# drprojects/DeepViewAgg

Measured on NVIDIA H100. Metric: Mpoints/s through view-agg fwd+bwd, higher is better.
Workload: dtype f32

## Files before the change

deepviewagg_b200/csrc/view_attention_lane.cu:

```cuda
#include "view_attention.cuh"

namespace dva {

constexpr int kLaneWarps = 4;
constexpr uint32_t kFull = 0xffffffffu;

struct LaneSmem {
  float wt[32][4];
  float at[32][4];
  float st[32][4];
  float Sp[32][4];
  float dq[32][4];
  uint32_t ri[32];
  uint32_t orow[32];
  uint32_t go[32];
  uint64_t bar;
  uint64_t pad;
};

template <typename T, int LPR>
__global__ void __launch_bounds__(kLaneWarps * 32, 5)
va_lane_bwd_kernel(const VAParams P, const int PR) {
  constexpr int VEC = Vec16<T>::N, RPI = 32 / LPR, CPE = LPR / 4, U = 4, RS = LPR * 16;
  extern __shared__ __align__(128) unsigned char rows_all[];
  __shared__ LaneSmem sm_all[kLaneWarps];
  const int warp = threadIdx.x >> 5, lane = threadIdx.x & 31;
  LaneSmem& sm = sm_all[warp];
  unsigned char* rows_s = rows_all + (size_t)warp * 32 * RS;
  const uint32_t rows_u = smem_u32(rows_s), bar_u = smem_u32(&sm.bar);
  uint32_t uses = 0;
  if (lane == 0) {
    mbar_init(bar_u, 1);
    mbar_init_fence();
  }
  __syncwarp();
  const int sg = lane / LPR, lir = lane % LPR, gk = lir / CPE;
  const uint32_t row_bytes = (uint32_t)P.C * sizeof(T);
  const char* __restrict__ xbase = reinterpret_cast<const char*>(P.x);
  const char* __restrict__ gob = reinterpret_cast<const char*>(P.gout) + lir * 16;
  char* __restrict__ gxb = reinterpret_cast<char*>(P.gx) + lir * 16;
  const bool gating = P.gate_w != nullptr;
  float4 gw4 = make_float4(0.f, 0.f, 0.f, 0.f), gb4 = gw4;
  if (gating) {
    gw4 = make_float4(P.gate_w[0], P.gate_w[1], P.gate_w[2], P.gate_w[3]);
    gb4 = make_float4(P.gate_b[0], P.gate_b[1], P.gate_b[2], P.gate_b[3]);
  }
  float4 dw4 = make_float4(0.f, 0.f, 0.f, 0.f), db4 = dw4;
  const bool scatter = P.scatter && P.idx != nullptr;

  auto issue_rows = [&](int nv, uint32_t rid) {
    fence_proxy_async();
    __syncwarp();
    if (lane == 0) mbar_expect_tx(bar_u, (uint32_t)nv * row_bytes);
    __syncwarp();
    if (lane < nv) bulk_g2s(rows_u + (uint32_t)lane * RS, xbase + (uint64_t)rid * row_bytes, row_bytes, bar_u);
  };
  auto wait_rows = [&]() {
    mbar_wait(bar_u, uses & 1u);
    ++uses;
  };

  auto rows_phase = [&](int nv, int64_t pg) {
    for (int u0 = 0; u0 < nv; u0 += RPI * U) {
      uint4 xr[U], gr[U];
      float w[U];
      uint32_t orow[U];
      bool ok[U];
#pragma unroll
      for (int q = 0; q < U; ++q) {
        const int u = u0 + q * RPI + sg;
        ok[q] = u < nv;
        const int uu = ok[q] ? u : 0;
        orow[q] = sm.orow[uu];
        w[q] = sm.wt[uu][gk];
        xr[q] = *reinterpret_cast<const uint4*>(rows_s + (size_t)uu * RS + lir * 16);
        gr[q] = *reinterpret_cast<const uint4*>(gob + (uint64_t)(pg + sm.go[uu]) * row_bytes);
      }
#pragma unroll
      for (int q = 0; q < U; ++q) {
        float fx[VEC], fg[VEC], dx[VEC];
        unpack16<T, VEC>(xr[q], fx);
        unpack16<T, VEC>(gr[q], fg);
        float dot = 0.f;
#pragma unroll
        for (int j = 0; j < VEC; ++j) {
          dot = fmaf(fg[j], fx[j], dot);
          dx[j] = w[q] * fg[j];
        }
        if (ok[q]) stg_stream16(gxb + (uint64_t)orow[q] * row_bytes, pack16<T, VEC>(dx));
#pragma unroll
        for (int o = 1; o < CPE; o <<= 1) dot += __shfl_xor_sync(kFull, dot, o);
        if (ok[q] && (lir & (CPE - 1)) == 0) sm.st[u0 + q * RPI + sg][gk] = dot;
      }
    }
  };

  const int64_t n_ranges = (P.N + PR - 1) / PR;
  const int64_t warps_total = (int64_t)gridDim.x * kLaneWarps;
  for (int64_t r = (int64_t)blockIdx.x * kLaneWarps + warp; r < n_ranges; r += warps_total) {
    const int64_t pa = r * PR;
    const int64_t pb = (pa + PR < P.N) ? pa + PR : P.N;
    for (int64_t pg = pa; pg < pb;) {
      const int64_t pk = pg + lane;
      const bool valid = pk < pb;
      const int64_t p0 = valid ? P.ptr[pk] : 0;
      const int cnt = valid ? (int)(P.ptr[pk + 1] - p0) : 0;
      int incl = cnt;
#pragma unroll
      for (int o = 1; o < 32; o <<= 1) {
        const int t = __shfl_up_sync(kFull, incl, o);
        if (lane >= o) incl += t;
      }
      const int excl = incl - cnt;
      const unsigned fitm = __ballot_sync(kFull, valid && incl <= 32);
      const int kfit = (fitm == kFull) ? 32 : __ffs(~fitm) - 1;
      const int64_t gvb = __shfl_sync(kFull, p0, 0);

      if (kfit == 0) {
        const int n = __shfl_sync(kFull, cnt, 0);
        const float4 smx = reinterpret_cast<const float4*>(P.s_max)[pg];
        const float4 sdn = reinterpret_cast<const float4*>(P.s_den)[pg];
        const int4 sar = reinterpret_cast<const int4*>(P.s_arg)[pg];
        const float inv_sq = P.group_scaling ? rsqrtf((float)n) : 1.f;
        float4 z4 = make_float4(1.f, 1.f, 1.f, 1.f), t4 = z4;
        if (gating) {
          z4 = gate_z4(gw4, smx, gb4);
          t4 = gate_t4(z4);
        }
        float4 Sacc = make_float4(0.f, 0.f, 0.f, 0.f);
        for (int c0 = 0; c0 < n; c0 += 32) {
          const int nv = (n - c0 < 32) ? n - c0 : 32;
          const int64_t v = gvb + c0 + lane;
          float4 a = make_float4(0.f, 0.f, 0.f, 0.f);
          __syncwarp();
          const uint32_t rid_l = lane < nv ? load_row_id(P.idx, P.idx64, v) : 0u;
          issue_rows(nv, rid_l);
          if (lane < nv) {
            const float4 c = __ldg(reinterpret_cast<const float4*>(P.compat) + v);
            a = make_float4(__expf((c.x - smx.x) * inv_sq) / sdn.x, __expf((c.y - smx.y) * inv_sq) / sdn.y,
                            __expf((c.z - smx.z) * inv_sq) / sdn.z, __expf((c.w - smx.w) * inv_sq) / sdn.w);
            sm.ri[lane] = rid_l;
            sm.orow[lane] = scatter ? rid_l : (uint32_t)v;
            sm.go[lane] = 0u;
            *reinterpret_cast<float4*>(sm.wt[lane]) = make_float4(a.x * t4.x, a.y * t4.y, a.z * t4.z, a.w * t4.w);
          }
          __syncwarp();
          wait_rows();
          rows_phase(nv, pg);
          __syncwarp();
          if (lane < nv) {
            const float4 raw = *reinterpret_cast<const float4*>(sm.st[lane]);
            const float4 sp = make_float4(raw.x * t4.x, raw.y * t4.y, raw.z * t4.z, raw.w * t4.w);
            Sacc.x = fmaf(a.x, sp.x, Sacc.x); Sacc.y = fmaf(a.y, sp.y, Sacc.y);
            Sacc.z = fmaf(a.z, sp.z, Sacc.z); Sacc.w = fmaf(a.w, sp.w, Sacc.w);
            reinterpret_cast<float4*>(P.gcompat)[v] = sp;
          }
        }
#pragma unroll
        for (int o = 16; o > 0; o >>= 1) {
          Sacc.x += __shfl_xor_sync(kFull, Sacc.x, o); Sacc.y += __shfl_xor_sync(kFull, Sacc.y, o);
          Sacc.z += __shfl_xor_sync(kFull, Sacc.z, o); Sacc.w += __shfl_xor_sync(kFull, Sacc.w, o);
        }
        float4 dq = make_float4(0.f, 0.f, 0.f, 0.f);
        if (gating) dq = gate_grad4(Sacc, z4, t4, gw4, smx, lane == 0, dw4, db4);
        __syncwarp();
        for (int c0 = lane; c0 < n; c0 += 32) {
          const int64_t v = gvb + c0;
          const float4 c = __ldg(reinterpret_cast<const float4*>(P.compat) + v);
          const float4 sp = __ldcg(reinterpret_cast<const float4*>(P.gcompat) + v);
          float4 d;
          d.x = __expf((c.x - smx.x) * inv_sq) / sdn.x * (sp.x - Sacc.x) * inv_sq;
          d.y = __expf((c.y - smx.y) * inv_sq) / sdn.y * (sp.y - Sacc.y) * inv_sq;
          d.z = __expf((c.z - smx.z) * inv_sq) / sdn.z * (sp.z - Sacc.z) * inv_sq;
          d.w = __expf((c.w - smx.w) * inv_sq) / sdn.w * (sp.w - Sacc.w) * inv_sq;
          if ((int)v == sar.x) d.x += dq.x;
          if ((int)v == sar.y) d.y += dq.y;
          if ((int)v == sar.z) d.z += dq.z;
          if ((int)v == sar.w) d.w += dq.w;
          reinterpret_cast<float4*>(P.gcompat)[v] = d;
        }
        pg += 1;
        continue;
      }

      const int nv = __shfl_sync(kFull, incl, kfit - 1);
      int mp = 0;
      for (int k = 0; k < kfit; ++k) {
        const int s = __shfl_sync(kFull, excl, k), c = __shfl_sync(kFull, cnt, k);
        if (lane >= s && lane < s + c) mp = k;
      }
      const int cntp = __shfl_sync(kFull, cnt, mp);
      float4 a = make_float4(0.f, 0.f, 0.f, 0.f), t4 = make_float4(1.f, 1.f, 1.f, 1.f);
      float inv_sq = 1.f;
      int4 sar = make_int4(-1, -1, -1, -1);
      const int64_t v = gvb + lane;
      __syncwarp();
      const uint32_t rid_m = lane < nv ? load_row_id(P.idx, P.idx64, v) : 0u;
      if (nv > 0) issue_rows(nv, rid_m);
      if (lane < nv) {
        const float4 c = __ldg(reinterpret_cast<const float4*>(P.compat) + v);
        const float4 smx = reinterpret_cast<const float4*>(P.s_max)[pg + mp];
        const float4 sdn = reinterpret_cast<const float4*>(P.s_den)[pg + mp];
        sar = reinterpret_cast<const int4*>(P.s_arg)[pg + mp];
        inv_sq = P.group_scaling ? rsqrtf((float)cntp) : 1.f;
        a = make_float4(__expf((c.x - smx.x) * inv_sq) / sdn.x, __expf((c.y - smx.y) * inv_sq) / sdn.y,
                        __expf((c.z - smx.z) * inv_sq) / sdn.z, __expf((c.w - smx.w) * inv_sq) / sdn.w);
        if (gating) t4 = gate_t4(gate_z4(gw4, smx, gb4));
        sm.ri[lane] = rid_m;
        sm.orow[lane] = scatter ? rid_m : (uint32_t)v;
        sm.go[lane] = (uint32_t)mp;
        *reinterpret_cast<float4*>(sm.at[lane]) = a;
        *reinterpret_cast<float4*>(sm.wt[lane]) = make_float4(a.x * t4.x, a.y * t4.y, a.z * t4.z, a.w * t4.w);
      }
      __syncwarp();

      if (nv > 0) wait_rows();
      rows_phase(nv, pg);
      __syncwarp();

      if (lane < nv) {
        float4 raw = *reinterpret_cast<const float4*>(sm.st[lane]);
        raw.x *= t4.x; raw.y *= t4.y; raw.z *= t4.z; raw.w *= t4.w;
        *reinterpret_cast<float4*>(sm.st[lane]) = raw;
      }
      __syncwarp();
      if (lane < kfit) {
        float4 S = make_float4(0.f, 0.f, 0.f, 0.f), dq = S;
        for (int j = 0; j < cnt; ++j) {
          const float4 aa = *reinterpret_cast<const float4*>(sm.at[excl + j]);
          const float4 sv = *reinterpret_cast<const float4*>(sm.st[excl + j]);
          S.x = fmaf(aa.x, sv.x, S.x); S.y = fmaf(aa.y, sv.y, S.y); S.z = fmaf(aa.z, sv.z, S.z); S.w = fmaf(aa.w, sv.w, S.w);
        }
        if (gating && cnt > 0) {
          const float4 smx = reinterpret_cast<const float4*>(P.s_max)[pk];
          const float4 z4 = gate_z4(gw4, smx, gb4);
          dq = gate_grad4(S, z4, gate_t4(z4), gw4, smx, true, dw4, db4);
        }
        *reinterpret_cast<float4*>(sm.Sp[lane]) = S;
        *reinterpret_cast<float4*>(sm.dq[lane]) = dq;
      }
      __syncwarp();
      if (lane < nv) {
        const float4 S = *reinterpret_cast<const float4*>(sm.Sp[mp]);
        const float4 dq = *reinterpret_cast<const float4*>(sm.dq[mp]);
        const float4 sv = *reinterpret_cast<const float4*>(sm.st[lane]);
        reinterpret_cast<float4*>(P.gcompat)[v] = compat_grad4(a, sv, S, inv_sq, (int)v, sar, dq);
      }
      pg += kfit;
    }
  }

  if (P.gate_partial != nullptr) store_gate_partial<kLaneWarps>(P.gate_partial, dw4, db4);
}

int va_lane_bwd(const VAParams& P, int dtype, int* grid_out, cudaStream_t st) {
  return with_dtype(dtype, [&](auto tag) {
    using T = decltype(tag);
    return with_lpr(P.C / Vec16<T>::N, [&](auto lpr) {
      constexpr int LPR = decltype(lpr)::value;
      auto kern = va_lane_bwd_kernel<T, LPR>;
      const size_t smem = (size_t)kLaneWarps * 32 * LPR * 16;
      int grid, pr;
      if (int rc = range_geometry(kern, smem, kLaneWarps, 8, 4, P.N, "va_lane_bwd", &grid, &pr)) return rc;
      kern<<<grid, kLaneWarps * 32, smem, st>>>(P, pr);
      *grid_out = grid;
      return check_launch("va_lane_bwd");
    });
  });
}

}
```

deepviewagg_b200/csrc/view_attention.cu:

```cuda
#include "view_attention.cuh"
#include <stdlib.h>

namespace dva {

#ifndef DVA_FWD_UNROLL
#define DVA_FWD_UNROLL 8
#endif
#ifndef DVA_BWD_UNROLL
#define DVA_BWD_UNROLL 4
#endif
#ifndef DVA_FWD_MINB
#define DVA_FWD_MINB 4
#endif
#ifndef DVA_BWD_MINB
#define DVA_BWD_MINB 4
#endif
constexpr int kWarps = 8;
constexpr int kUnroll = DVA_FWD_UNROLL;
constexpr int kUnrollBwd = DVA_BWD_UNROLL;

template <typename T, int VEC> struct Chunk {
  uint4 raw;
  __device__ __forceinline__ void load(const void* p) { raw = ldg_stream16(p); }
  __device__ __forceinline__ void zero() { raw = make_uint4(0u, 0u, 0u, 0u); }
// ... 319 lines not shown
        if (single_tile) {
          gk[k] = gk0[k]; off[k] = off0[k]; live[k] = live0[k];
        } else {
          const int c0 = ct + (lir + LPR * k) * VEC;
          live[k] = c0 < C;
          const int cc = live[k] ? c0 : 0;
          gk[k] = group_of_channel(cc, C, G);
          off[k] = (uint32_t)cc * sizeof(T);
        }
        const float tk = __shfl_sync(0xffffffffu, t, gk[k]);
        load_chunk<T, VEC>(gob + i * (int64_t)row_bytes + off[k], gd[k]);
#pragma unroll
        for (int j = 0; j < VEC; ++j) gd[k][j] = live[k] ? gd[k][j] * tk : 0.f;
      }
    };
    if (single_tile) load_gd(0);

    for (int vs = 0; vs < n; vs += 32) {
      const int nc = min(32, n - vs);
      __syncwarp();
      for (int e = lane; e < nc * G; e += 32) {
        const int slot = gl * kTileStride + e / G;
        att_s[slot] = expf((__ldg(cp + vs * G + e) - m) * inv_sq) * inv_den;
        if (!assign_s) s_s[slot] = 0.f;
      }
      if (lane < nc) {
        const uint32_t lin = (uint32_t)(p0 + vs + lane);
        const uint32_t r = has_idx ? (uint32_t)load_idx(P.idx, P.idx64, p0 + vs + lane) : lin;
        row_s[lane] = r;
        orow_s[lane] = scatter ? r : lin;
      }
      __syncwarp();

      for (int ct = 0; ct < C; ct += TILE_C) {
        if (!single_tile) load_gd(ct);
        const uint32_t* rs = row_s + sg;
        const uint32_t* os = orow_s + sg;
        const float* as[CPL]; float* ss[CPL];
        const char* xk[CPL]; char* ok_[CPL];
#pragma unroll
        for (int k = 0; k < CPL; ++k) {
          as[k] = att_s + gk[k] * kTileStride + sg;
          ss[k] = s_s + gk[k] * kTileStride + sg;
          xk[k] = xb + off[k];
          ok_[k] = gxb + off[k];
        }

        auto consume = [&](int v0, const Chunk<T, VEC> (&f)[CPL], bool ok) {
          const uint32_t orow = os[v0];
#pragma unroll
          for (int k = 0; k < CPL; ++k) {
            float fv[VEC], dx[VEC];
            f[k].get(fv);
            const float a = as[k][v0];
            float dot = 0.f;
#pragma unroll
            for (int j = 0; j < VEC; ++j) {
              dot = fmaf(gd[k][j], fv[j], dot);
              dx[j] = a * gd[k][j];
            }
            const bool lv = ok && live[k];
            if (lv) store_chunk<T, VEC>(row_addr(ok_[k], orow, row_bytes), dx);
            if constexpr (REG) {
              float r = dot;
#pragma unroll
              for (int b = 0; (1 << b) < LPR; ++b)
                r = fmaf(__shfl_xor_sync(0xffffffffu, r, 1 << b), red_mask[b], r);
              if (lv && leader) {
                if (assign_s) ss[k][v0] = r; else ss[k][v0] += r;
              }
            } else {
              for (int g = 0; g < G; ++g) {
                const bool mine = lv && (gk[k] == g);
                if (!__any_sync(0xffffffffu, mine)) continue;
                float r = mine ? dot : 0.f;
#pragma unroll
                for (int o = 1; o < LPR; o <<= 1) r += __shfl_xor_sync(0xffffffffu, r, o);
                if (ok && lir == 0) s_s[g * kTileStride + sg + v0] += r;
              }
            }
          }
        };

        int v0 = 0;
        for (; v0 + RPI * U <= nc; v0 += RPI * U) {
          Chunk<T, VEC> f[U][CPL];
#pragma unroll
          for (int u = 0; u < U; ++u) {
            const uint32_t srow = rs[v0 + u * RPI];
#pragma unroll
            for (int k = 0; k < CPL; ++k) f[u][k].load(row_addr(xk[k], srow, row_bytes));
          }
#pragma unroll
          for (int u = 0; u < U; ++u) consume(v0 + u * RPI, f[u], true);
        }
        for (; v0 < nc; v0 += RPI * UT) {
          Chunk<T, VEC> f[UT][CPL];
          bool okv[UT];
#pragma unroll
          for (int u = 0; u < UT; ++u) {
            okv[u] = v0 + u * RPI + sg < nc;
            if (v0 + u * RPI < nc) {
              const uint32_t srow = okv[u] ? rs[v0 + u * RPI] : row_s[0];
#pragma unroll
              for (int k = 0; k < CPL; ++k) f[u][k].load(row_addr(xk[k], srow, row_bytes));
            }
          }
#pragma unroll
          for (int u = 0; u < UT; ++u)
            if (v0 + u * RPI < nc) consume(okv[u] ? v0 + u * RPI : 0 - sg, f[u], okv[u]);
        }
        __syncwarp();
      }

      for (int e = lane; e < nc * G; e += 32) {
        const int slot = gl * kTileStride + e / G;
        const float sv = s_s[slot];
        S = fmaf(att_s[slot], sv, S);
        if (!one_chunk) gc[vs * G + e] = sv;
      }
    }

    S = group_lane_sum(S, G);
    const float one_m_t2 = 1.f - t * t;
    const float dLdt = (t != 0.f) ? S / t : 0.f;
    const bool open = gating && z > 0.f;
    const float dq = open ? dLdt * one_m_t2 * gw : 0.f;
    if (open && lane < G) {
      dw_acc += dLdt * one_m_t2 * m;
      db_acc += dLdt * one_m_t2;
    }
    for (int e = lane; e < nG; e += 32) {
      float a, sv;
      if (one_chunk) { const int slot = gl * kTileStride + e / G; a = att_s[slot]; sv = s_s[slot]; }
      else { a = expf((__ldg(cp + e) - m) * inv_sq) * inv_den; sv = gc[e]; }
      gc[e] = compat_grad(a, sv, S, inv_sq, p0 + e / G == arg_v, dq);
    }
  }

  if (P.gate_partial != nullptr) {
    if (lane < G) {
      gate_s[(warp * 2 + 0) * G + lane] = dw_acc;
      gate_s[(warp * 2 + 1) * G + lane] = db_acc;
    }
    __syncthreads();
    if (threadIdx.x < 2 * G) {
      float acc = 0.f;
      for (int w = 0; w < kWarps; ++w) acc += gate_s[w * 2 * G + threadIdx.x];
      P.gate_partial[(int64_t)blockIdx.x * 2 * G + threadIdx.x] = acc;
    }
  }
}

__global__ void gate_reduce_kernel(const float* __restrict__ partial, float* __restrict__ out,
                                   int blocks, int twoG) {
  const int lane = threadIdx.x & 31;
  for (int j = threadIdx.x >> 5; j < twoG; j += blockDim.x >> 5) {
    float acc = 0.f;
    for (int b = lane; b < blocks; b += 32) acc += partial[(int64_t)b * twoG + j];
#pragma unroll
    for (int o = 16; o > 0; o >>= 1) acc += __shfl_xor_sync(0xffffffffu, acc, o);
    if (lane == 0) out[j] = acc;
  }
}

struct VAConfig { int vec, lpr, cpl; bool reg; };

template <typename T>
static VAConfig choose_config(const VAParams& P, const void* o1, const void* o2, bool need_regular) {
  constexpr int V16 = Vec16<T>::N;
  const int C = P.C, G = P.G;
  bool vec_ok = (C % V16 == 0) && aligned16(P.x) && aligned16(o1) && (o2 == nullptr || aligned16(o2));
  if (vec_ok) {
    for (int c0 = 0; c0 < C && vec_ok; c0 += V16)
      if (group_of_channel(c0, C, G) != group_of_channel(c0 + V16 - 1, C, G)) vec_ok = false;
  }
  auto regular = [&](int vec) {
    if (C % G != 0 || (C / G) % vec != 0) return false;
    const int cpg = (C / G) / vec;
    return (cpg & (cpg - 1)) == 0;
  };
  if (vec_ok && need_regular && !regular(V16)) vec_ok = false;
  VAConfig cfg;
  if (!vec_ok) { cfg.vec = 1; cfg.lpr = 32; cfg.cpl = (C > 32) ? 4 : 1; cfg.reg = regular(1); return cfg; }
  const int cv = C / V16;
  cfg.vec = V16; cfg.reg = true;
  if (cv <= 4) { cfg.lpr = 4; cfg.cpl = 1; }
  else if (cv <= 8) { cfg.lpr = 8; cfg.cpl = 1; }
  else if (cv <= 16) { cfg.lpr = 16; cfg.cpl = 1; }
  else if (cv <= 32) { cfg.lpr = 32; cfg.cpl = 1; }
  else if (cv <= 64) { cfg.lpr = 32; cfg.cpl = 2; }
  else { cfg.lpr = 32; cfg.cpl = 4; }
  return cfg;
}

template <typename K>
static int va_grid(K kern, size_t smem, int64_t N) {
  int occ = 0;
  if (cudaOccupancyMaxActiveBlocksPerMultiprocessor(&occ, kern, kWarps * 32, smem) != cudaSuccess || occ < 1) occ = 2;
  int64_t blocks = (int64_t)kNumSMs * occ;
  const int64_t need = (N + kWarps - 1) / kWarps;
  if (blocks > need) blocks = need;
  if (blocks < 1) blocks = 1;
  return (int)blocks;
}

constexpr int kMinBlocksFwd = DVA_FWD_MINB;
constexpr int kMinBlocksBwd = DVA_BWD_MINB;

static size_t fwd_smem(int G) {
  return (size_t)kWarps * G * kTileStride * sizeof(float) + (size_t)kWarps * 32 * sizeof(uint32_t);
}
static size_t bwd_smem(int G) {
  return (size_t)2 * kWarps * G * kTileStride * sizeof(float) + (size_t)kWarps * 64 * sizeof(uint32_t) +
         (size_t)kWarps * 2 * G * sizeof(float);
}

template <typename T, int VEC, int LPR, int CPL>
static int launch_fwd(const VAParams& P, cudaStream_t st) {
  const size_t smem = fwd_smem(P.G);
  auto kern = view_attention_fwd_kernel<T, VEC, LPR, CPL, (CPL >= 4 ? 2 : kMinBlocksFwd)>;
  (void)smem_opt_in(kern, smem);
  kern<<<va_grid(kern, smem, P.N), kWarps * 32, smem, st>>>(P);
  return check_launch("view_attention_fwd");
}

template <typename T, int VEC, int LPR, int CPL, bool REG>
static int launch_bwd_k(const VAParams& P, int* grid_out, cudaStream_t st) {
  const size_t smem = bwd_smem(P.G);
  auto kern = view_attention_bwd_kernel<T, VEC, LPR, CPL, (CPL >= 4 ? 2 : kMinBlocksBwd), REG>;
  (void)smem_opt_in(kern, smem);
  const int grid = va_grid(kern, smem, P.N);
  *grid_out = grid;
  kern<<<grid, kWarps * 32, smem, st>>>(P);
  return check_launch("view_attention_bwd");
}

template <typename T, int VEC, int LPR, int CPL>
static int launch_bwd(const VAParams& P, bool reg, int* grid_out, cudaStream_t st) {
  if constexpr (VEC == 1) {
    if (!reg) return launch_bwd_k<T, VEC, LPR, CPL, false>(P, grid_out, st);
  }
  return launch_bwd_k<T, VEC, LPR, CPL, true>(P, grid_out, st);
}

template <typename T, typename F> static bool with_config(const VAConfig& cfg, F&& f) {
  return with_value<321, 324, 1041, 1081, 1161, 1321, 1322, 1324>(
      (cfg.vec == 1 ? 0 : 1000) + cfg.lpr * 10 + cfg.cpl, [&](auto code) {
        constexpr int c = decltype(code)::value;
        f(std::integral_constant<int, c >= 1000 ? Vec16<T>::N : 1>{}, std::integral_constant<int, c % 1000 / 10>{},
          std::integral_constant<int, c % 10>{});
      });
}

template <typename T> static int fwd_typed(const VAParams& P, cudaStream_t st) {
  int rc = DVA_OK;
  if (!with_config<T>(choose_config<T>(P, P.out, nullptr, false), [&](auto vec, auto lpr, auto cpl) {
        rc = launch_fwd<T, decltype(vec)::value, decltype(lpr)::value, decltype(cpl)::value>(P, st);
      }))
    return fail(DVA_EUNSUPPORTED, "view_attention_fwd: no kernel for this row layout");
  return rc;
}
template <typename T> static int bwd_typed(const VAParams& P, int* grid, cudaStream_t st) {
  const VAConfig cfg = choose_config<T>(P, P.gout, P.gx, true);
  int rc = DVA_OK;
  if (!with_config<T>(cfg, [&](auto vec, auto lpr, auto cpl) {
        rc = launch_bwd<T, decltype(vec)::value, decltype(lpr)::value, decltype(cpl)::value>(P, cfg.reg, grid, st);
      }))
    return fail(DVA_EUNSUPPORTED, "view_attention_bwd: no kernel for this row layout");
  return rc;
}

template <typename T>
static bool short_rows_ok(const VAParams& P, const void* o1, const void* o2) {
  constexpr int V16 = Vec16<T>::N;
  const int C = P.C, G = P.G;
  if (G != 4) return false;
  if (C % V16 != 0 || C / V16 > 32) return false;
  if (!aligned16(P.x) || !aligned16(o1) || (o2 != nullptr && !aligned16(o2))) return false;
  if (!aligned16(P.compat)) return false;
  if (P.V >= (1ll << 31) || P.R >= (1ll << 32)) return false;
  for (int c0 = 0; c0 < C; c0 += V16)
    if (group_of_channel(c0, C, G) != group_of_channel(c0 + V16 - 1, C, G)) return false;
  return true;
}
static bool ring_fwd_applicable(const VAParams& P, int dtype) {
  if (!with_dtype(dtype, [&](auto tag) { return short_rows_ok<decltype(tag)>(P, P.out, nullptr); })) return false;
  if (P.att != nullptr && !aligned16(P.att)) return false;
  if (P.seg_max != nullptr && (!aligned16(P.seg_max) || !aligned16(P.seg_den) || !aligned16(P.seg_arg))) return false;
  return true;
}
static bool short_bwd_applicable(const VAParams& P, int dtype) {
  return with_dtype(dtype, [&](auto tag) {
    using T = decltype(tag);
    constexpr int V16 = Vec16<T>::N;
    if (!short_rows_ok<T>(P, P.gout, P.gx)) return false;
    if (P.C % P.G != 0 || (P.C / P.G) % V16 != 0) return false;
    const int cpg = (P.C / P.G) / V16;
    if ((cpg & (cpg - 1)) != 0) return false;
    return aligned16(P.s_max) && aligned16(P.s_den) && aligned16(P.s_arg) && aligned16(P.gcompat);
  });
}

static bool pow2_le32(int64_t g) { return g >= 1 && g <= 32 && (g & (g - 1)) == 0; }

static std::atomic<int>& va_path() {
  static std::atomic<int> p{[] {
    const char* e = getenv("DVA_VA_PATH");
    if (e == nullptr) return 0;
    if (strcmp(e, "stream") == 0) return 1;
    if (strcmp(e, "ring") == 0) return 2;
    if (strcmp(e, "lane") == 0) return 3;
    return 0;
  }()};
  return p;
}

#ifndef DVA_RING_MAX_MEAN_VIEWS
#define DVA_RING_MAX_MEAN_VIEWS 12
#endif
static bool use_ring(const VAParams& P, int dtype, bool applicable, bool backward) {
  if (!applicable) return false;
  const int path = va_path().load(std::memory_order_relaxed);
  if (path == 1 || path == 3) return false;
  if (path == 2) return true;
  if (P.V > (int64_t)DVA_RING_MAX_MEAN_VIEWS * P.N) return false;
  const size_t esz = dtype == DVA_F32 ? 4 : 2;
  return !backward || ((size_t)P.C * esz > 128 && (size_t)P.C * esz <= 512);
}

static bool use_lane_bwd(const VAParams& P, bool applicable) {
  if (!applicable) return false;
  const int path = va_path().load(std::memory_order_relaxed);
  return path == 0 || path == 3;
}

}

using namespace dva;

extern "C" int dva_view_attention_fwd(const void* x, const void* idx, int idx_is_i64,
                                      const float* compat, const int64_t* ptr,
                                      const float* gate_w, const float* gate_b, void* out,
                                      float* att, float* seg_max, float* seg_den,
                                      int32_t* seg_arg, int64_t N, int64_t V, int64_t R,
                                      int64_t C, int64_t G, int group_scaling, float eps,
                                      int dtype, void* stream) {
  if (N < 0 || V < 0 || R < 0 || C < 1 || G < 1) return fail(DVA_EINVAL, "view_attention_fwd: bad sizes");
  if (G > C) return fail(DVA_EINVAL, "view_attention_fwd: num_groups > channels");
  if (!pow2_le32(G)) return fail(DVA_EUNSUPPORTED, "view_attention_fwd: G must be a power of two <= 32");
  if (C > (1 << 20)) return fail(DVA_EUNSUPPORTED, "view_attention_fwd: C too large");
  if (R >= (1ll << 32) || V >= (1ll << 32)) return fail(DVA_EUNSUPPORTED, "view_attention_fwd: more than 2^32 rows");
  if (N == 0) return DVA_OK;
  if (!ptr || !out || (V > 0 && (!x || !compat))) return fail(DVA_EINVAL, "view_attention_fwd: null pointer");
  if ((gate_w == nullptr) != (gate_b == nullptr)) return fail(DVA_EINVAL, "view_attention_fwd: gate_w/gate_b must both be given");
  if ((seg_max != nullptr) && (!seg_den || !seg_arg)) return fail(DVA_EINVAL, "view_attention_fwd: seg_max/seg_den/seg_arg go together");
  if (idx == nullptr && R < V) return fail(DVA_EINVAL, "view_attention_fwd: identity idx needs R >= V");
  VAParams P{};
  P.x = x; P.idx = idx; P.idx64 = idx_is_i64; P.compat = compat; P.ptr = ptr;
  P.gate_w = gate_w; P.gate_b = gate_b; P.out = out; P.att = att;
  P.seg_max = seg_max; P.seg_den = seg_den; P.seg_arg = seg_arg;
  P.N = N; P.V = V; P.R = R; P.C = (int)C; P.G = (int)G; P.group_scaling = group_scaling; P.eps = eps;
  cudaStream_t st = (cudaStream_t)stream;
  if (!known_dtype(dtype)) return fail(DVA_EINVAL, "view_attention_fwd: unknown dtype");
  if (use_ring(P, dtype, ring_fwd_applicable(P, dtype), false)) return va_ring_fwd(P, dtype, st);
  return with_dtype(dtype, [&](auto tag) { return fwd_typed<decltype(tag)>(P, st); });
}

extern "C" int dva_view_attention_set_path(int path) {
  if (path < 0 || path > 3) return fail(DVA_EINVAL, "view_attention_set_path: 0 = auto, 1 = streaming, 2 = ring, 3 = lane (backward)");
  va_path().store(path, std::memory_order_relaxed);
  return DVA_OK;
}

extern "C" size_t dva_view_attention_bwd_workspace_bytes(int64_t G) {
  return (size_t)kNumSMs * 8 * 2 * (size_t)(G > 0 ? G : 1) * sizeof(float);
}

extern "C" int dva_view_attention_bwd(const void* x, const void* idx, int idx_is_i64,
                                      const float* compat, const int64_t* ptr,
                                      const float* gate_w, const float* gate_b,
                                      const void* grad_out, const float* seg_max,
                                      const float* seg_den, const int32_t* seg_arg,
                                      void* grad_x_rows, float* grad_compat, float* grad_gate,
                                      int scatter_rows, int64_t N, int64_t V, int64_t R,
                                      int64_t C, int64_t G, int group_scaling, int dtype,
                                      void* workspace, size_t workspace_bytes, void* stream) {
  if (N < 0 || V < 0 || R < 0 || C < 1 || G < 1) return fail(DVA_EINVAL, "view_attention_bwd: bad sizes");
  if (G > C) return fail(DVA_EINVAL, "view_attention_bwd: num_groups > channels");
  if (!pow2_le32(G)) return fail(DVA_EUNSUPPORTED, "view_attention_bwd: G must be a power of two <= 32");
  if (R >= (1ll << 32) || V >= (1ll << 32)) return fail(DVA_EUNSUPPORTED, "view_attention_bwd: more than 2^32 rows");
  const bool gating = gate_w != nullptr;
  if (gating != (gate_b != nullptr)) return fail(DVA_EINVAL, "view_attention_bwd: gate_w/gate_b must both be given");
  cudaStream_t st = (cudaStream_t)stream;
  if (N == 0 || V == 0) {
    if (gating && grad_gate) cudaMemsetAsync(grad_gate, 0, 2 * G * sizeof(float), st);
    return DVA_OK;
  }
  if (!x || !compat || !ptr || !grad_out || !seg_max || !seg_den || !seg_arg || !grad_x_rows || !grad_compat)
    return fail(DVA_EINVAL, "view_attention_bwd: null pointer");
  if (gating && (!grad_gate || !workspace || workspace_bytes < dva_view_attention_bwd_workspace_bytes(G)))
    return fail(DVA_EINVAL, "view_attention_bwd: gating needs grad_gate and workspace");
  VAParams P{};
  P.x = x; P.idx = idx; P.idx64 = idx_is_i64; P.compat = compat; P.ptr = ptr;
  P.gate_w = gate_w; P.gate_b = gate_b; P.gout = grad_out;
  P.s_max = seg_max; P.s_den = seg_den; P.s_arg = seg_arg;
  P.gx = grad_x_rows; P.gcompat = grad_compat; P.scatter = scatter_rows;
  P.gate_partial = gating ? reinterpret_cast<float*>(workspace) : nullptr;
  P.N = N; P.V = V; P.R = R; P.C = (int)C; P.G = (int)G; P.group_scaling = group_scaling;
  int grid = 1;
  int rc;
  if (!known_dtype(dtype)) return fail(DVA_EINVAL, "view_attention_bwd: unknown dtype");
  const bool short_rows = short_bwd_applicable(P, dtype);
  if (use_ring(P, dtype, short_rows, true)) {
    rc = va_ring_bwd(P, dtype, &grid, st);
  } else if (use_lane_bwd(P, short_rows)) {
    rc = va_lane_bwd(P, dtype, &grid, st);
  } else {
    rc = with_dtype(dtype, [&](auto tag) { return bwd_typed<decltype(tag)>(P, &grid, st); });
  }
  if (rc) return rc;
  if (gating) {
    gate_reduce_kernel<<<1, 1024, 0, st>>>(P.gate_partial, grad_gate, grid, 2 * (int)G);
    return check_launch("gate_reduce");
  }
  return DVA_OK;
}
```

deepviewagg_b200/csrc/view_attention.cuh:

```cuda
#pragma once
#include "dva_common.cuh"

namespace dva {

struct VAParams {
  const void* x; const void* idx; int idx64;
  const float* compat; const int64_t* ptr;
  const float* gate_w; const float* gate_b;
  void* out; float* att; float* seg_max; float* seg_den; int32_t* seg_arg;
  const void* gout; const float* s_max; const float* s_den; const int32_t* s_arg;
  void* gx; float* gcompat; float* gate_partial; int scatter;
  int64_t N, V, R;
  int C, G, group_scaling;
  float eps;
};

constexpr int kTileStride = 33;

__device__ __forceinline__ float group_lane_sum(float v, int G) {
  for (int off = 16; off >= G; off >>= 1) v += __shfl_xor_sync(0xffffffffu, v, off);
  return v;
}

__device__ __forceinline__ uint32_t smem_u32(const void* p) { return (uint32_t)__cvta_generic_to_shared(p); }
__device__ __forceinline__ void mbar_init(uint32_t bar, uint32_t count) {
  asm volatile("mbarrier.init.shared::cta.b64 [%0], %1;" ::"r"(bar), "r"(count) : "memory");
}
__device__ __forceinline__ void mbar_init_fence() { asm volatile("fence.mbarrier_init.release.cluster;" ::: "memory"); }
__device__ __forceinline__ void mbar_expect_tx(uint32_t bar, uint32_t bytes) {
  asm volatile("mbarrier.arrive.expect_tx.shared::cta.b64 _, [%0], %1;" ::"r"(bar), "r"(bytes) : "memory");
}
__device__ __forceinline__ void mbar_wait(uint32_t bar, uint32_t parity) {
  uint32_t ok = 0;
  while (!ok) {
    asm volatile(
        "{ .reg .pred p; mbarrier.try_wait.parity.shared::cta.b64 p, [%1], %2; selp.u32 %0, 1, 0, p; }"
        : "=r"(ok) : "r"(bar), "r"(parity) : "memory");
  }
}
__device__ __forceinline__ void bulk_g2s(uint32_t dst, const void* src, uint32_t bytes, uint32_t bar) {
  asm volatile("cp.async.bulk.shared::cluster.global.mbarrier::complete_tx::bytes [%0], [%1], %2, [%3];"
               ::"r"(dst), "l"(src), "r"(bytes), "r"(bar) : "memory");
}
__device__ __forceinline__ void fence_proxy_async() { asm volatile("fence.proxy.async.shared::cta;" ::: "memory"); }

__device__ __forceinline__ uint32_t load_row_id(const void* idx, int idx64, int64_t v) {
  if (idx == nullptr) return (uint32_t)v;
  return idx64 ? (uint32_t) reinterpret_cast<const int64_t*>(idx)[v]
               : (uint32_t) reinterpret_cast<const int32_t*>(idx)[v];
}
__device__ __forceinline__ float sel4(const float4& v, int g) {
  return g == 0 ? v.x : (g == 1 ? v.y : (g == 2 ? v.z : v.w));
}

__device__ __forceinline__ float gate_t(float z) { return tanhf(fmaxf(z, 0.f)); }
__device__ __forceinline__ float4 gate_z4(const float4& w, const float4& m, const float4& b) {
  return make_float4(fmaf(w.x, m.x, b.x), fmaf(w.y, m.y, b.y), fmaf(w.z, m.z, b.z), fmaf(w.w, m.w, b.w));
}
__device__ __forceinline__ float4 gate_t4(const float4& z) {
  return make_float4(gate_t(z.x), gate_t(z.y), gate_t(z.z), gate_t(z.w));
}

__device__ __forceinline__ float gate_grad(float S, float z, float t, float w, float m, bool keep, float& dw,
                                           float& db) {
  if (!(z > 0.f)) return 0.f;
  const float dLdt = (t != 0.f) ? S / t : 0.f;
  const float u = dLdt * (1.f - t * t);
  const float dq = u * w;
  if (keep) {
    dw += u * m;
    db += u;
  }
  return dq;
}
__device__ __forceinline__ float4 gate_grad4(const float4& S, const float4& z, const float4& t, const float4& w,
                                             const float4& m, bool keep, float4& dw, float4& db) {
  return make_float4(gate_grad(S.x, z.x, t.x, w.x, m.x, keep, dw.x, db.x),
                     gate_grad(S.y, z.y, t.y, w.y, m.y, keep, dw.y, db.y),
                     gate_grad(S.z, z.z, t.z, w.z, m.z, keep, dw.z, db.z),
                     gate_grad(S.w, z.w, t.w, w.w, m.w, keep, dw.w, db.w));
}

__device__ __forceinline__ float compat_grad(float a, float sv, float S, float inv_sq, bool is_arg, float dq) {
  float d = a * (sv - S) * inv_sq;
  if (is_arg) d += dq;
  return d;
}
__device__ __forceinline__ float4 compat_grad4(const float4& a, const float4& sv, const float4& S, float inv_sq,
                                               int v, const int4& arg, const float4& dq) {
  return make_float4(compat_grad(a.x, sv.x, S.x, inv_sq, v == arg.x, dq.x),
                     compat_grad(a.y, sv.y, S.y, inv_sq, v == arg.y, dq.y),
                     compat_grad(a.z, sv.z, S.z, inv_sq, v == arg.z, dq.z),
                     compat_grad(a.w, sv.w, S.w, inv_sq, v == arg.w, dq.w));
}

template <int WARPS>
__device__ __forceinline__ void store_gate_partial(float* __restrict__ partial, const float4& dw, const float4& db) {
  __shared__ float gate_s[WARPS][8];
  const int warp = threadIdx.x >> 5, lane = threadIdx.x & 31;
  float v[8] = {dw.x, dw.y, dw.z, dw.w, db.x, db.y, db.z, db.w};
#pragma unroll
  for (int q = 0; q < 8; ++q) {
#pragma unroll
    for (int o = 16; o > 0; o >>= 1) v[q] += __shfl_xor_sync(0xffffffffu, v[q], o);
  }
  if (lane == 0) {
#pragma unroll
    for (int q = 0; q < 8; ++q) gate_s[warp][q] = v[q];
  }
  __syncthreads();
  if ((int)threadIdx.x < 8) {
    float acc = 0.f;
    for (int w = 0; w < WARPS; ++w) acc += gate_s[w][threadIdx.x];
    partial[(int64_t)blockIdx.x * 8 + threadIdx.x] = acc;
  }
}

template <typename K>
int range_geometry(K kern, size_t smem, int warps_per_cta, int max_ctas_per_sm, int ranges_per_warp, int64_t N,
                   const char* what, int* grid_out, int* pr_out) {
  cudaError_t e = cudaFuncSetAttribute(kern, cudaFuncAttributeMaxDynamicSharedMemorySize, (int)smem);
  if (e != cudaSuccess) return failf((int)e, "%s: %zu bytes of shared memory: %s", what, smem, cudaGetErrorString(e));
  int occ = 0;
  if (cudaOccupancyMaxActiveBlocksPerMultiprocessor(&occ, kern, warps_per_cta * 32, smem) != cudaSuccess || occ < 1) occ = 1;
  if (occ > max_ctas_per_sm) occ = max_ctas_per_sm;
  int64_t grid = (int64_t)kNumSMs * occ;
  const int64_t slots = grid * warps_per_cta * ranges_per_warp;
  int64_t pr = (N + slots - 1) / slots;
  if (pr < 8) pr = 8;
  const int64_t n_ranges = (N + pr - 1) / pr;
  const int64_t need = (n_ranges + warps_per_cta - 1) / warps_per_cta;
  if (grid > need) grid = need;
  if (grid < 1) grid = 1;
  *grid_out = (int)grid; *pr_out = (int)pr;
  return DVA_OK;
}

int va_ring_fwd(const VAParams& P, int dtype, cudaStream_t st);
int va_ring_bwd(const VAParams& P, int dtype, int* grid_out, cudaStream_t st);
int va_lane_bwd(const VAParams& P, int dtype, int* grid_out, cudaStream_t st);

}
```

Baseline: 53.04.

## Hoist single-group gout row load and shrink lane-backward shared memory

When all rows in a chunk belong to one group (long-group path or kfit==1), the gout row is loaded once into registers instead of reloaded per row inside the rows loop. The per-group S and dq broadcast moves from shared-memory staging to warp shuffles, and unused smem arrays (ri, Sp, dq, go writes) are removed. Launch bounds drop to 3 CTAs/SM for LPR==32 to allow more registers, with a static_assert checking smem fits. This trades occupancy for register headroom at wide rows and adds a templated rows_phase variant.

```diff
diff --git a/deepviewagg_b200/csrc/view_attention_lane.cu b/deepviewagg_b200/csrc/view_attention_lane.cu
--- a/deepviewagg_b200/csrc/view_attention_lane.cu
+++ b/deepviewagg_b200/csrc/view_attention_lane.cu
@@ -9,17 +9,18 @@
   float wt[32][4];
   float at[32][4];
   float st[32][4];
-  float Sp[32][4];
-  float dq[32][4];
-  uint32_t ri[32];
   uint32_t orow[32];
   uint32_t go[32];
   uint64_t bar;
   uint64_t pad;
 };
 
+constexpr size_t kLaneCtaSmem512 =
+    (size_t)kLaneWarps * 32 * 512 + kLaneWarps * sizeof(LaneSmem) + kLaneWarps * 8 * sizeof(float) + 1024;
+static_assert(3 * kLaneCtaSmem512 <= 228 * 1024, "lane backward: 3 CTAs per SM no longer fit at 512-byte rows");
+
 template <typename T, int LPR>
-__global__ void __launch_bounds__(kLaneWarps * 32, 5)
+__global__ void __launch_bounds__(kLaneWarps * 32, LPR == 32 ? 3 : 5)
 va_lane_bwd_kernel(const VAParams P, const int PR) {
   constexpr int VEC = Vec16<T>::N, RPI = 32 / LPR, CPE = LPR / 4, U = 4, RS = LPR * 16;
   extern __shared__ __align__(128) unsigned char rows_all[];
@@ -60,9 +61,10 @@
     ++uses;
   };
 
-  auto rows_phase = [&](int nv, int64_t pg) {
+  auto rows_phase = [&](int nv, int64_t pg, auto one, const uint4& g1) {
+    constexpr bool ONE = decltype(one)::value;
     for (int u0 = 0; u0 < nv; u0 += RPI * U) {
-      uint4 xr[U], gr[U];
+      uint4 xr[U], gr[ONE ? 1 : U];
       float w[U];
       uint32_t orow[U];
       bool ok[U];
@@ -74,13 +76,13 @@
         orow[q] = sm.orow[uu];
         w[q] = sm.wt[uu][gk];
         xr[q] = *reinterpret_cast<const uint4*>(rows_s + (size_t)uu * RS + lir * 16);
-        gr[q] = *reinterpret_cast<const uint4*>(gob + (uint64_t)(pg + sm.go[uu]) * row_bytes);
+        if (!ONE) gr[q] = *reinterpret_cast<const uint4*>(gob + (uint64_t)(pg + sm.go[uu]) * row_bytes);
       }
 #pragma unroll
       for (int q = 0; q < U; ++q) {
         float fx[VEC], fg[VEC], dx[VEC];
         unpack16<T, VEC>(xr[q], fx);
-        unpack16<T, VEC>(gr[q], fg);
+        unpack16<T, VEC>(ONE ? g1 : gr[ONE ? 0 : q], fg);
         float dot = 0.f;
 #pragma unroll
         for (int j = 0; j < VEC; ++j) {
@@ -127,6 +129,7 @@
           z4 = gate_z4(gw4, smx, gb4);
           t4 = gate_t4(z4);
         }
+        const uint4 g1 = *reinterpret_cast<const uint4*>(gob + (uint64_t)pg * row_bytes);
         float4 Sacc = make_float4(0.f, 0.f, 0.f, 0.f);
         for (int c0 = 0; c0 < n; c0 += 32) {
           const int nv = (n - c0 < 32) ? n - c0 : 32;
@@ -139,14 +142,12 @@
             const float4 c = __ldg(reinterpret_cast<const float4*>(P.compat) + v);
             a = make_float4(__expf((c.x - smx.x) * inv_sq) / sdn.x, __expf((c.y - smx.y) * inv_sq) / sdn.y,
                             __expf((c.z - smx.z) * inv_sq) / sdn.z, __expf((c.w - smx.w) * inv_sq) / sdn.w);
-            sm.ri[lane] = rid_l;
             sm.orow[lane] = scatter ? rid_l : (uint32_t)v;
-            sm.go[lane] = 0u;
             *reinterpret_cast<float4*>(sm.wt[lane]) = make_float4(a.x * t4.x, a.y * t4.y, a.z * t4.z, a.w * t4.w);
           }
           __syncwarp();
           wait_rows();
-          rows_phase(nv, pg);
+          rows_phase(nv, pg, std::true_type{}, g1);
           __syncwarp();
           if (lane < nv) {
             const float4 raw = *reinterpret_cast<const float4*>(sm.st[lane]);
@@ -197,6 +198,8 @@
       __syncwarp();
       const uint32_t rid_m = lane < nv ? load_row_id(P.idx, P.idx64, v) : 0u;
       if (nv > 0) issue_rows(nv, rid_m);
+      uint4 g1 = make_uint4(0u, 0u, 0u, 0u);
+      if (kfit == 1) g1 = *reinterpret_cast<const uint4*>(gob + (uint64_t)pg * row_bytes);
       if (lane < nv) {
         const float4 c = __ldg(reinterpret_cast<const float4*>(P.compat) + v);
         const float4 smx = reinterpret_cast<const float4*>(P.s_max)[pg + mp];
@@ -206,7 +209,6 @@
         a = make_float4(__expf((c.x - smx.x) * inv_sq) / sdn.x, __expf((c.y - smx.y) * inv_sq) / sdn.y,
                         __expf((c.z - smx.z) * inv_sq) / sdn.z, __expf((c.w - smx.w) * inv_sq) / sdn.w);
         if (gating) t4 = gate_t4(gate_z4(gw4, smx, gb4));
-        sm.ri[lane] = rid_m;
         sm.orow[lane] = scatter ? rid_m : (uint32_t)v;
         sm.go[lane] = (uint32_t)mp;
         *reinterpret_cast<float4*>(sm.at[lane]) = a;
@@ -215,7 +217,8 @@
       __syncwarp();
 
       if (nv > 0) wait_rows();
-      rows_phase(nv, pg);
+      if (kfit == 1) rows_phase(nv, pg, std::true_type{}, g1);
+      else rows_phase(nv, pg, std::false_type{}, g1);
       __syncwarp();
 
       if (lane < nv) {
@@ -224,8 +227,8 @@
         *reinterpret_cast<float4*>(sm.st[lane]) = raw;
       }
       __syncwarp();
+      float4 S = make_float4(0.f, 0.f, 0.f, 0.f), dq = S;
       if (lane < kfit) {
-        float4 S = make_float4(0.f, 0.f, 0.f, 0.f), dq = S;
         for (int j = 0; j < cnt; ++j) {
           const float4 aa = *reinterpret_cast<const float4*>(sm.at[excl + j]);
           const float4 sv = *reinterpret_cast<const float4*>(sm.st[excl + j]);
@@ -236,13 +239,12 @@
           const float4 z4 = gate_z4(gw4, smx, gb4);
           dq = gate_grad4(S, z4, gate_t4(z4), gw4, smx, true, dw4, db4);
         }
-        *reinterpret_cast<float4*>(sm.Sp[lane]) = S;
-        *reinterpret_cast<float4*>(sm.dq[lane]) = dq;
-      }
-      __syncwarp();
+      }
+      S.x = __shfl_sync(kFull, S.x, mp); S.y = __shfl_sync(kFull, S.y, mp);
+      S.z = __shfl_sync(kFull, S.z, mp); S.w = __shfl_sync(kFull, S.w, mp);
+      dq.x = __shfl_sync(kFull, dq.x, mp); dq.y = __shfl_sync(kFull, dq.y, mp);
+      dq.z = __shfl_sync(kFull, dq.z, mp); dq.w = __shfl_sync(kFull, dq.w, mp);
       if (lane < nv) {
-        const float4 S = *reinterpret_cast<const float4*>(sm.Sp[mp]);
-        const float4 dq = *reinterpret_cast<const float4*>(sm.dq[mp]);
         const float4 sv = *reinterpret_cast<const float4*>(sm.st[lane]);
         reinterpret_cast<float4*>(P.gcompat)[v] = compat_grad4(a, sv, S, inv_sq, (int)v, sar, dq);
       }
```

New measurement: 53.73, median of 6. +1.3%, better.

## Prefetch next segment metadata and hold grad-out rows in lane bwd for long segments

Applied to the files above, without the earlier changes.

Adds a long-segment mode to the lane backward kernel. For G=4, 512-byte rows and many views per point, it software-prefetches the next group's ptr, row ids and compat values while the current group is processed. When a warp handles a single segment, it loads the grad-out row once and reuses it for all views. It also moves the Sp/dq scratch into the row staging buffer to cut per-warp shared memory, and lowers min blocks for LPR=32 so the compiler has more registers. A standalone HBM bandwidth probe kernel is added as well. Reusing the staging buffer for Sp/dq depends on those rows no longer being needed at that point.

```diff
diff --git a/deepviewagg_b200/csrc/hbm_probe.cu b/deepviewagg_b200/csrc/hbm_probe.cu
--- /dev/null
+++ b/deepviewagg_b200/csrc/hbm_probe.cu
@@ -0,0 +1,93 @@
+#include "dva_common.cuh"
+#include "../../include/dva_probe.h"
+
+namespace dva_probe {
+
+constexpr int kWarps = 8;
+constexpr uint32_t kRowBytes = 512;
+enum { kSeqRead = DVA_PROBE_SEQ_READ, kGather = DVA_PROBE_GATHER, kGatherWrite = DVA_PROBE_GATHER_WRITE, kCopy = DVA_PROBE_COPY };
+
+template <int MIX, int U>
+__global__ void __launch_bounds__(kWarps * 32)
+hbm_mix_kernel(const char* __restrict__ x, const int32_t* __restrict__ idx, char* __restrict__ y, int64_t rows,
+               uint32_t* __restrict__ sink) {
+  constexpr bool kIndexed = MIX == kGather || MIX == kGatherWrite;
+  constexpr bool kWrites = MIX == kGatherWrite || MIX == kCopy;
+  const int lane = threadIdx.x & 31;
+  const int64_t units = rows / 32;
+  const int64_t nw = (int64_t)gridDim.x * kWarps;
+  const char* xl = x + lane * 16;
+  char* yl = y + lane * 16;
+  uint32_t acc = 0;
+  int64_t u = (int64_t)blockIdx.x * kWarps + (threadIdx.x >> 5);
+  uint32_t r_next = 0;
+  if (kIndexed && u < units) r_next = (uint32_t)idx[u * 32 + lane];
+  for (; u < units; u += nw) {
+    const int64_t v0 = u * 32;
+    const uint32_t r = kIndexed ? r_next : (uint32_t)(v0 + lane);
+    if (kIndexed && u + nw < units) r_next = (uint32_t)idx[(u + nw) * 32 + lane];
+#pragma unroll 1
+    for (int s = 0; s < 32; s += U) {
+      uint4 d[U];
+#pragma unroll
+      for (int q = 0; q < U; ++q) {
+        const uint32_t row = __shfl_sync(0xffffffffu, r, s + q);
+        d[q] = dva::ldg_stream16(xl + (uint64_t)row * kRowBytes);
+      }
+#pragma unroll
+      for (int q = 0; q < U; ++q) {
+        if constexpr (kWrites) dva::stg_stream16(yl + (uint64_t)(v0 + s + q) * kRowBytes, d[q]);
+        else acc ^= d[q].x ^ d[q].y ^ d[q].z ^ d[q].w;
+      }
+    }
+  }
+  if (!kWrites && acc == 0x9e3779b9u) sink[0] = acc;
+}
+
+template <int MIX, int U>
+static int launch(const void* x, const int32_t* idx, void* y, int64_t rows, int ctas_per_sm, uint32_t* sink,
+                  int* ctas_out, cudaStream_t st) {
+  auto kern = hbm_mix_kernel<MIX, U>;
+  int occ = 0;
+  if (cudaOccupancyMaxActiveBlocksPerMultiprocessor(&occ, kern, kWarps * 32, 0) != cudaSuccess || occ < 1) occ = 1;
+  const int ctas = ctas_per_sm < occ ? ctas_per_sm : occ;
+  kern<<<dva::kNumSMs * ctas, kWarps * 32, 0, st>>>(reinterpret_cast<const char*>(x), idx,
+                                                     reinterpret_cast<char*>(y), rows, sink);
+  *ctas_out = ctas;
+  return dva::check_launch("hbm_probe");
+}
+
+template <int MIX>
+static int launch_u(int u, const void* x, const int32_t* idx, void* y, int64_t rows, int ctas_per_sm,
+                    uint32_t* sink, int* ctas_out, cudaStream_t st) {
+  switch (u) {
+    case 2: return launch<MIX, 2>(x, idx, y, rows, ctas_per_sm, sink, ctas_out, st);
+    case 4: return launch<MIX, 4>(x, idx, y, rows, ctas_per_sm, sink, ctas_out, st);
+    case 8: return launch<MIX, 8>(x, idx, y, rows, ctas_per_sm, sink, ctas_out, st);
+    default: return launch<MIX, 16>(x, idx, y, rows, ctas_per_sm, sink, ctas_out, st);
+  }
+}
+
+}
+
+using namespace dva_probe;
+
+extern "C" int dva_probe_hbm_mix(int mix, const void* x, const int32_t* idx, void* y, int64_t rows,
+                                 int rows_per_warp, int ctas_per_sm, uint32_t* sink, int* ctas_out, void* stream) {
+  if (mix < kSeqRead || mix > kCopy) return dva::fail(DVA_EINVAL, "probe_hbm_mix: unknown mix");
+  if (rows_per_warp != 2 && rows_per_warp != 4 && rows_per_warp != 8 && rows_per_warp != 16)
+    return dva::fail(DVA_EINVAL, "probe_hbm_mix: rows_per_warp must be 2, 4, 8 or 16");
+  if (ctas_per_sm < 1 || ctas_per_sm > 8) return dva::fail(DVA_EINVAL, "probe_hbm_mix: ctas_per_sm must be 1 .. 8");
+  if (rows < 32 || rows % 32 != 0 || rows >= (1ll << 32)) return dva::fail(DVA_EINVAL, "probe_hbm_mix: rows must be a multiple of 32 below 2^32");
+  if (!x || !sink || !ctas_out || ((mix == kGather || mix == kGatherWrite) && !idx) ||
+      ((mix == kGatherWrite || mix == kCopy) && !y))
+    return dva::fail(DVA_EINVAL, "probe_hbm_mix: null pointer");
+  if (!dva::aligned16(x) || (y && !dva::aligned16(y))) return dva::fail(DVA_EALIGN, "probe_hbm_mix: rows must be 16-byte aligned");
+  cudaStream_t st = (cudaStream_t)stream;
+  switch (mix) {
+    case kSeqRead: return launch_u<kSeqRead>(rows_per_warp, x, idx, y, rows, ctas_per_sm, sink, ctas_out, st);
+    case kGather: return launch_u<kGather>(rows_per_warp, x, idx, y, rows, ctas_per_sm, sink, ctas_out, st);
+    case kGatherWrite: return launch_u<kGatherWrite>(rows_per_warp, x, idx, y, rows, ctas_per_sm, sink, ctas_out, st);
+    default: return launch_u<kCopy>(rows_per_warp, x, idx, y, rows, ctas_per_sm, sink, ctas_out, st);
+  }
+}
diff --git a/deepviewagg_b200/csrc/view_attention.cu b/deepviewagg_b200/csrc/view_attention.cu
--- a/deepviewagg_b200/csrc/view_attention.cu
+++ b/deepviewagg_b200/csrc/view_attention.cu
@@ -645,6 +645,10 @@
   });
 }
 
+static bool long_seg_shape(const VAParams& P, int dtype) {
+  return P.G == 4 && (int64_t)P.C * (dtype == DVA_F32 ? 4 : 2) == 512 && P.V >= (int64_t)kLongSegMeanViews * P.N;
+}
+
 static bool pow2_le32(int64_t g) { return g >= 1 && g <= 32 && (g & (g - 1)) == 0; }
 
 static std::atomic<int>& va_path() {
@@ -758,6 +762,7 @@
   if (use_ring(P, dtype, short_rows, true)) {
     rc = va_ring_bwd(P, dtype, &grid, st);
   } else if (use_lane_bwd(P, short_rows)) {
+    P.long_seg = long_seg_shape(P, dtype);
     rc = va_lane_bwd(P, dtype, &grid, st);
   } else {
     rc = with_dtype(dtype, [&](auto tag) { return bwd_typed<decltype(tag)>(P, &grid, st); });
diff --git a/deepviewagg_b200/csrc/view_attention.cuh b/deepviewagg_b200/csrc/view_attention.cuh
--- a/deepviewagg_b200/csrc/view_attention.cuh
+++ b/deepviewagg_b200/csrc/view_attention.cuh
@@ -10,12 +10,14 @@
   void* out; float* att; float* seg_max; float* seg_den; int32_t* seg_arg;
   const void* gout; const float* s_max; const float* s_den; const int32_t* s_arg;
   void* gx; float* gcompat; float* gate_partial; int scatter;
+  int long_seg;
   int64_t N, V, R;
   int C, G, group_scaling;
   float eps;
 };
 
 constexpr int kTileStride = 33;
+constexpr int kLongSegMeanViews = 24;
 
 __device__ __forceinline__ float group_lane_sum(float v, int G) {
   for (int off = 16; off >= G; off >>= 1) v += __shfl_xor_sync(0xffffffffu, v, off);
diff --git a/deepviewagg_b200/csrc/view_attention_lane.cu b/deepviewagg_b200/csrc/view_attention_lane.cu
--- a/deepviewagg_b200/csrc/view_attention_lane.cu
+++ b/deepviewagg_b200/csrc/view_attention_lane.cu
@@ -9,9 +9,6 @@
   float wt[32][4];
   float at[32][4];
   float st[32][4];
-  float Sp[32][4];
-  float dq[32][4];
-  uint32_t ri[32];
   uint32_t orow[32];
   uint32_t go[32];
   uint64_t bar;
@@ -19,7 +16,7 @@
 };
 
 template <typename T, int LPR>
-__global__ void __launch_bounds__(kLaneWarps * 32, 5)
+__global__ void __launch_bounds__(kLaneWarps * 32, LPR == 32 ? 3 : 5)
 va_lane_bwd_kernel(const VAParams P, const int PR) {
   constexpr int VEC = Vec16<T>::N, RPI = 32 / LPR, CPE = LPR / 4, U = 4, RS = LPR * 16;
   extern __shared__ __align__(128) unsigned char rows_all[];
@@ -27,6 +24,8 @@
   const int warp = threadIdx.x >> 5, lane = threadIdx.x & 31;
   LaneSmem& sm = sm_all[warp];
   unsigned char* rows_s = rows_all + (size_t)warp * 32 * RS;
+  float* Sp = reinterpret_cast<float*>(rows_s);
+  float* dqp = Sp + 32 * 4;
   const uint32_t rows_u = smem_u32(rows_s), bar_u = smem_u32(&sm.bar);
   uint32_t uses = 0;
   if (lane == 0) {
@@ -60,7 +59,7 @@
     ++uses;
   };
 
-  auto rows_phase = [&](int nv, int64_t pg) {
+  auto rows_phase = [&](int nv, int64_t pg, bool hold, const uint4& g_hold) {
     for (int u0 = 0; u0 < nv; u0 += RPI * U) {
       uint4 xr[U], gr[U];
       float w[U];
@@ -74,7 +73,8 @@
         orow[q] = sm.orow[uu];
         w[q] = sm.wt[uu][gk];
         xr[q] = *reinterpret_cast<const uint4*>(rows_s + (size_t)uu * RS + lir * 16);
-        gr[q] = *reinterpret_cast<const uint4*>(gob + (uint64_t)(pg + sm.go[uu]) * row_bytes);
+        gr[q] = hold ? g_hold
+                     : *reinterpret_cast<const uint4*>(gob + (uint64_t)(pg + sm.go[uu]) * row_bytes);
       }
 #pragma unroll
       for (int q = 0; q < U; ++q) {
@@ -94,6 +94,13 @@
       }
     }
   };
+
+  const bool long_seg = LPR == 32 && P.long_seg;
+  const uint4 g_none = make_uint4(0u, 0u, 0u, 0u);
+  int64_t pf_pg = -1, pf_v = -1, pf_p0 = 0;
+  int pf_cnt = 0;
+  uint32_t pf_rid = 0u;
+  float4 pf_c = make_float4(0.f, 0.f, 0.f, 0.f);
 
   const int64_t n_ranges = (P.N + PR - 1) / PR;
   const int64_t warps_total = (int64_t)gridDim.x * kLaneWarps;
@@ -103,8 +110,9 @@
     for (int64_t pg = pa; pg < pb;) {
       const int64_t pk = pg + lane;
       const bool valid = pk < pb;
-      const int64_t p0 = valid ? P.ptr[pk] : 0;
-      const int cnt = valid ? (int)(P.ptr[pk + 1] - p0) : 0;
+      const bool pf = long_seg && pf_pg == pg;
+      const int64_t p0 = pf ? pf_p0 : (valid ? P.ptr[pk] : 0);
+      const int cnt = pf ? pf_cnt : (valid ? (int)(P.ptr[pk + 1] - p0) : 0);
       int incl = cnt;
 #pragma unroll
       for (int o = 1; o < 32; o <<= 1) {
@@ -139,14 +147,13 @@
             const float4 c = __ldg(reinterpret_cast<const float4*>(P.compat) + v);
             a = make_float4(__expf((c.x - smx.x) * inv_sq) / sdn.x, __expf((c.y - smx.y) * inv_sq) / sdn.y,
                             __expf((c.z - smx.z) * inv_sq) / sdn.z, __expf((c.w - smx.w) * inv_sq) / sdn.w);
-            sm.ri[lane] = rid_l;
             sm.orow[lane] = scatter ? rid_l : (uint32_t)v;
             sm.go[lane] = 0u;
             *reinterpret_cast<float4*>(sm.wt[lane]) = make_float4(a.x * t4.x, a.y * t4.y, a.z * t4.z, a.w * t4.w);
           }
           __syncwarp();
           wait_rows();
-          rows_phase(nv, pg);
+          rows_phase(nv, pg, false, g_none);
           __syncwarp();
           if (lane < nv) {
             const float4 raw = *reinterpret_cast<const float4*>(sm.st[lane]);
@@ -195,10 +202,24 @@
       int4 sar = make_int4(-1, -1, -1, -1);
       const int64_t v = gvb + lane;
       __syncwarp();
-      const uint32_t rid_m = lane < nv ? load_row_id(P.idx, P.idx64, v) : 0u;
+      const bool pfv = long_seg && pf_v == gvb;
+      const uint32_t rid_m = lane < nv ? (pfv ? pf_rid : load_row_id(P.idx, P.idx64, v)) : 0u;
       if (nv > 0) issue_rows(nv, rid_m);
+      const bool hold = long_seg && kfit == 1;
+      const uint4 g_hold = hold ? *reinterpret_cast<const uint4*>(gob + (uint64_t)pg * row_bytes) : g_none;
+      const float4 c_m = (lane < nv && pfv) ? pf_c : make_float4(0.f, 0.f, 0.f, 0.f);
+      if (long_seg && pg + kfit < pb) {
+        const int64_t q = pg + kfit + lane;
+        pf_pg = pg + kfit;
+        pf_p0 = q < pb ? P.ptr[q] : 0;
+        pf_cnt = q < pb ? (int)(P.ptr[q + 1] - pf_p0) : 0;
+        pf_v = gvb + nv;
+        const int64_t w = pf_v + lane;
+        pf_rid = w < P.V ? load_row_id(P.idx, P.idx64, w) : 0u;
+        pf_c = w < P.V ? __ldg(reinterpret_cast<const float4*>(P.compat) + w) : make_float4(0.f, 0.f, 0.f, 0.f);
+      }
       if (lane < nv) {
-        const float4 c = __ldg(reinterpret_cast<const float4*>(P.compat) + v);
+        const float4 c = pfv ? c_m : __ldg(reinterpret_cast<const float4*>(P.compat) + v);
         const float4 smx = reinterpret_cast<const float4*>(P.s_max)[pg + mp];
         const float4 sdn = reinterpret_cast<const float4*>(P.s_den)[pg + mp];
         sar = reinterpret_cast<const int4*>(P.s_arg)[pg + mp];
@@ -206,7 +227,6 @@
         a = make_float4(__expf((c.x - smx.x) * inv_sq) / sdn.x, __expf((c.y - smx.y) * inv_sq) / sdn.y,
                         __expf((c.z - smx.z) * inv_sq) / sdn.z, __expf((c.w - smx.w) * inv_sq) / sdn.w);
         if (gating) t4 = gate_t4(gate_z4(gw4, smx, gb4));
-        sm.ri[lane] = rid_m;
         sm.orow[lane] = scatter ? rid_m : (uint32_t)v;
         sm.go[lane] = (uint32_t)mp;
         *reinterpret_cast<float4*>(sm.at[lane]) = a;
@@ -215,7 +235,7 @@
       __syncwarp();
 
       if (nv > 0) wait_rows();
-      rows_phase(nv, pg);
+      rows_phase(nv, pg, hold, g_hold);
       __syncwarp();
 
       if (lane < nv) {
@@ -236,13 +256,13 @@
           const float4 z4 = gate_z4(gw4, smx, gb4);
           dq = gate_grad4(S, z4, gate_t4(z4), gw4, smx, true, dw4, db4);
         }
-        *reinterpret_cast<float4*>(sm.Sp[lane]) = S;
-        *reinterpret_cast<float4*>(sm.dq[lane]) = dq;
+        *reinterpret_cast<float4*>(Sp + 4 * lane) = S;
+        *reinterpret_cast<float4*>(dqp + 4 * lane) = dq;
       }
       __syncwarp();
       if (lane < nv) {
-        const float4 S = *reinterpret_cast<const float4*>(sm.Sp[mp]);
-        const float4 dq = *reinterpret_cast<const float4*>(sm.dq[mp]);
+        const float4 S = *reinterpret_cast<const float4*>(Sp + 4 * mp);
+        const float4 dq = *reinterpret_cast<const float4*>(dqp + 4 * mp);
         const float4 sv = *reinterpret_cast<const float4*>(sm.st[lane]);
         reinterpret_cast<float4*>(P.gcompat)[v] = compat_grad4(a, sv, S, inv_sq, (int)v, sar, dq);
       }
diff --git a/include/dva_probe.h b/include/dva_probe.h
--- /dev/null
+++ b/include/dva_probe.h
@@ -0,0 +1,17 @@
+#ifndef DVA_PROBE_H_
+#define DVA_PROBE_H_
+
+#include <stdint.h>
+
+#ifdef __cplusplus
+extern "C" {
+#endif
+
+enum { DVA_PROBE_SEQ_READ = 0, DVA_PROBE_GATHER = 1, DVA_PROBE_GATHER_WRITE = 2, DVA_PROBE_COPY = 3 };
+int dva_probe_hbm_mix(int mix, const void* x, const int32_t* idx, void* y, int64_t rows, int rows_per_warp,
+                      int ctas_per_sm, uint32_t* sink, int* ctas_out, void* stream);
+
+#ifdef __cplusplus
+}
+#endif
+#endif
```

Measured after the change: 54.20 before, 54.89 after (median of 6 runs). +1.3%, better.
